# xiph/LPCNet

Hardware: AMD Instinct MI355X
Metric: 16 kHz samples/sec & concurrent real-time streams, 1/2/4/8 MI355X (higher is better)
Workload: dtype f32; 1 GPU; 2048 concurrent streams (each with its own feature file) per GPU x 25 frames (4000 samples) per step, fp32 weights, register-resident block-sparse GRU-A, bit-exact (PARITY) arithmetic; eight streams per CU as two groups of four half a step apart (BASELINE config 2's 1024 streams fill half of these stream slots: `also.config2_1024_streams`); arithmetic=parity, gru_a_blocks=1382, gru_a_densities=0.05,0.05,0.2 (benchmark model), gru_a_items_per_lane=30, streams_per_gpu=2048, streams_per_workgroup=8

## Files before the change

lpcnet_amd/csrc/sample_common.hip.h:

```cpp
#pragma once
#include <hip/hip_runtime.h>
#include <stdint.h>
#include "lpcnet_engine.h"
#include "lpcnet_math.h"

namespace lpcn {

constexpr int NA = LPCN_N_A, NB = LPCN_N_B, RA = LPCN_ROWS_A, RB = LPCN_ROWS_B;

#define LPCN_GLOBAL __attribute__((address_space(1)))
template <typename T> __device__ __forceinline__ const LPCN_GLOBAL T *as_global(const T *p)
{
    return (const LPCN_GLOBAL T *)(uintptr_t)p;
}
template <typename T> __device__ __forceinline__ LPCN_GLOBAL T *as_global_rw(T *p)
{
    return (LPCN_GLOBAL T *)(uintptr_t)p;
}
#define LPCN_REMAT_V(x) asm volatile("" : "+v"(x))
#define LPCN_REMAT_S(x) asm volatile("" : "+s"(x))

__device__ __forceinline__ uint32_t lds_addr(const void *ptr)
{
    return (uint32_t)(uintptr_t)(__attribute__((address_space(3))) unsigned char *)(unsigned char *)ptr;
}
__device__ __forceinline__ void lds_publish(const uint32_t addr, const int seq)
{
    asm volatile("ds_write_b32 %0, %1" :: "v"(addr), "v"(seq) : "memory");
}
__device__ __forceinline__ void lds_arrive(const uint32_t addr)
{
    int one = 1;
    unsigned long long ex;
    asm volatile("s_mov_b64 %0, exec\n\t"
                 "s_mov_b64 exec, 1\n\t"
                 "ds_add_u32 %1, %2\n\t"
                 "s_mov_b64 exec, %0"
                 : "=&s"(ex) : "v"(addr), "v"(one) : "memory");
}
template <bool SLEEP> __device__ __forceinline__ void lds_poll_until(const uint32_t addr, const int want)
{
    int v;
    do {
        asm volatile("ds_read_b32 %0, %1\n\ts_waitcnt lgkmcnt(0)" : "=v"(v) : "v"(addr) : "memory");
        v = __builtin_amdgcn_readfirstlane(v);
        if (SLEEP && v != want) __builtin_amdgcn_s_sleep(1);
    } while (v != want);
}


template <int J> __device__ __forceinline__ float row_bcast(float v)
{
    return __builtin_bit_cast(float, __builtin_amdgcn_update_dpp(0, __builtin_bit_cast(int, v), 0x150 + J, 0xf, 0xf, false));
}
template <int J> __device__ __forceinline__ float lpc_chain(float r, float prod)
{
    if constexpr (J < LPCN_LPC_ORDER) return lpc_chain<J + 1>(r - row_bcast<J>(prod), prod);
    else return r;
}
__device__ __forceinline__ float row_shr1(float v, float fill)
{
    return __builtin_bit_cast(float, __builtin_amdgcn_update_dpp(__builtin_bit_cast(int, fill), __builtin_bit_cast(int, v), 0x111, 0xf, 0xf, false));
}

struct LeaderCells {
    float *lead;
    int *idx;
    float *thr;
    short *pcm;
};

template <int S> __device__ __forceinline__ void open_sample(const LeaderCells &c, const int tid0, const bool live, const float newest, const float prod, const int exc, const bool per_frame)
{
    int t_ = tid0;
    LPCN_REMAT_V(t_);
    const int lrow = (t_ & 63) >> 4, tap = t_ & 15;
    const float r = lpc_chain<0>(0.f, prod);
    const int u = lpcn_lin2ulaw((tap & 1) ? r : newest);
    const int u_pred = __builtin_amdgcn_mov_dpp(u, 0xB1, 0xf, 0xf, true);
    if (tap == 0) {
        if (live) {
            c.lead[lrow * 8 + 0] = r;
            c.idx[lrow] = u | (u_pred << 8) | (exc << 16);
        } else {
            c.idx[lrow] = 0;
        }
        if (per_frame) c.idx[S + lrow] = live ? 1 : 0;
    }
}

__device__ __forceinline__ void draw_thresholds(const LeaderCells &c, const float *logit_tab, const int ls)
{
    int *li = (int *)c.lead + ls * 8;
    uint32_t rng[4] = {(uint32_t)li[4], (uint32_t)li[5], (uint32_t)li[6], (uint32_t)li[7]};
    const uint32_t r0 = lpcn_kiss99(rng), r1 = lpcn_kiss99(rng);
    li[4] = (int)rng[0]; li[5] = (int)rng[1]; li[6] = (int)rng[2]; li[7] = (int)rng[3];
#pragma unroll
    for (int b = 0; b < 4; ++b) {
        c.thr[ls * 8 + b] = logit_tab[(r0 >> (8 * b)) & 0xFF];
        c.thr[ls * 8 + 4 + b] = logit_tab[(r1 >> (8 * b)) & 0xFF];
    }
}

__device__ __forceinline__ int tree_walk(const unsigned long long *mask_row)
{
    typedef unsigned u4 __attribute__((ext_vector_type(4)));
    const u4 *mk = (const u4 *)mask_row;
    const u4 qa = mk[0], qb = mk[1], qc = mk[2], qd = mk[3];
    auto bit_of = [](unsigned word, int k) { return (int)((word >> (2 * k)) & 1u); };
    int val = 0;
#pragma unroll
    for (int b = 0; b < 4; ++b) val = (val << 1) | bit_of(qa[0], (1 << b) | val);
    val = (val << 1) | bit_of(qa[1], val);
    val = (val << 1) | bit_of((val & 16) ? qa[3] : qa[2], val & 15);
    {
        const int k = val >> 4;
        const unsigned lo = (k & 1) ? qb[1] : qb[0], hi = (k & 1) ? qb[3] : qb[2];
        val = (val << 1) | bit_of((k & 2) ? hi : lo, val & 15);
    }
    {
        const int k = val >> 4;
        const unsigned a0 = (k & 1) ? qc[1] : qc[0], a1 = (k & 1) ? qc[3] : qc[2];
        const unsigned a2 = (k & 1) ? qd[1] : qd[0], a3 = (k & 1) ? qd[3] : qd[2];
        const unsigned b0 = (k & 2) ? a1 : a0, b1 = (k & 2) ? a3 : a2;
        val = (val << 1) | bit_of((k & 4) ? b1 : b0, val & 15);
    }
    return val;
}

__device__ __forceinline__ void draw_sample(const LeaderCells &c, const unsigned long long *mask_row, const float *ulaw_tab, const int lrow, const int tap,
                                            const bool live, const int smp, const int preload, float &hist, float &pcm, float &deemph, int &exc)
{
    pcm = 0.f; deemph = 0.f; exc = 0;
    if (live) {
        const float pred = c.lead[lrow * 8 + 0];
        deemph = c.lead[lrow * 8 + 1];
        exc = tree_walk(mask_row);
        if (smp < preload) {
            const float x = (float)c.pcm[lrow * LPCN_FRAME_SIZE + smp];
            exc = lpcn_lin2ulaw(x - 0.85f * deemph - pred);
            pcm = x - 0.85f * deemph;
        } else {
            pcm = pred + ulaw_tab[exc];
        }
    }
    {
        const float shifted = row_shr1(hist, pcm);
        hist = live ? shifted : hist;
    }
    if (tap == 0 && live) ((int *)c.lead)[lrow * 8 + 2] = exc;
}
__device__ __forceinline__ void finish_sample(const LeaderCells &c, const int lrow, const int tap, const bool live, const int smp, const int preload, float pcm, const float deemph)
{
    if (tap == 0) {
        if (live) {
            pcm = pcm + 0.85f * deemph;
            c.lead[lrow * 8 + 1] = pcm;
            if (smp >= preload) c.pcm[lrow * LPCN_FRAME_SIZE + smp] = (short)lpcn_round_pcm(pcm);
        } else {
            c.pcm[lrow * LPCN_FRAME_SIZE + smp] = 0;
        }
    }
}
__device__ __forceinline__ bool stream_is_live(const LpcnSampleArgs *Ap, const LPCN_GLOBAL lpcn_stream_state *states, const int stream, const int f)
{
    const int fc_ref = Ap->fc_base ? as_global(Ap->fc_base)[stream] : states[stream].frame_count;
    int fc = Ap->fc_advance ? fc_ref + f + 1 : fc_ref;
    if (fc > 1000) fc = 1000;
    return fc > LPCN_FEATURES_DELAY;
}

template <class L> __device__ __forceinline__ void stage_tables(unsigned char *smem, const LpcnSampleArgs *Ap, const int tid, const int brec_dwords)
{
    const auto *t0 = as_global(Ap->tab_tansig), *t1 = as_global(Ap->tab_ulaw2lin), *t2 = as_global(Ap->tab_logit);
    for (int i = tid; i < 201; i += LPCN_WG_THREADS) ((float *)(smem + L::tansig))[i] = t0[i];
    for (int i = tid; i < 256; i += LPCN_WG_THREADS) {
        ((float *)(smem + L::ulaw))[i] = t1[i];
        ((float *)(smem + L::logit))[i] = t2[i];
    }
    const auto *ab1 = as_global(Ap->a_bias1), *adg = as_global(Ap->a_diag);
    for (int i = tid; i < RA; i += LPCN_WG_THREADS) {
        ((float *)(smem + L::abias))[2 * i] = ab1[i];
        ((float *)(smem + L::abias))[2 * i + 1] = adg[i];
    }
    const auto *br = as_global(Ap->b_rec), *bb = as_global(Ap->b_bias);
    for (int i = tid; i < brec_dwords; i += LPCN_WG_THREADS) ((uint32_t *)(smem + L::brec))[i] = ((const LPCN_GLOBAL uint32_t *)br)[i];
    for (int i = tid; i < 2 * RB; i += LPCN_WG_THREADS) ((float *)(smem + L::bbias))[i] = bb[i];
    if (tid < 7) ((int *)(smem + L::bstart))[tid] = as_global(Ap->b_start)[tid];
}
#define LPCN_GRUB_SHIFT 0x321100
__device__ __forceinline__ void stage_grub_weights(unsigned char *bw, const LpcnSampleArgs *Ap, const int tid, const bool shifted)
{
    const int nb_b = Ap->nb_b;
    const auto *src = (const LPCN_GLOBAL uint32_t *)as_global(Ap->b_w);
    for (int i = tid; i < (nb_b + 8) * 32; i += LPCN_WG_THREADS) {
        int di = i;
        if (shifted) {
            if (i < nb_b * 32) di = i + ((LPCN_GRUB_SHIFT >> (4 * ((i >> 5) / 96))) & 15) * 32;
            else if (i < (nb_b + 5) * 32) di = i + 3 * 32;
            else continue;
        }
        ((uint32_t *)bw)[di] = i < nb_b * 32 ? src[i] : 0u;
    }
}
__device__ __forceinline__ void stage_leader_record(const LeaderCells &c, const int s, const LPCN_GLOBAL lpcn_stream_state *st)
{
    c.idx[s] = 0;
    c.lead[s * 8 + 0] = 0.f;
    c.lead[s * 8 + 1] = st->deemph_mem;
    ((int *)c.lead)[s * 8 + 2] = st->last_exc;
#pragma unroll
    for (int j = 0; j < 4; ++j) ((uint32_t *)c.lead)[s * 8 + 4 + j] = st->rng[j];
}
}
```

lpcnet_amd/csrc/sample_kernel_x2.hip.h:

```cpp
#pragma once
#include "sample_kernel.hip.h"

namespace lpcn {

#define LPCN_X2_LW 4
#define LPCN_X2_TW 0
#define LPCN_X2_HG 10

struct LdsX2 {
    static constexpr int S = 4;
    static constexpr int HA_STRIDE = 16 * S;
    static constexpr int g_hA    = 0;
    static constexpr int g_hT    = g_hA + 96 * HA_STRIDE + 24 * 16;
    static constexpr int g_prec  = g_hT + NA * S * 4;
    static constexpr int g_hB    = g_prec + NA * S * 4;
    static constexpr int g_idx   = g_hB + S * NB * 4;
    static constexpr int g_thr   = g_idx + S * 16;
    static constexpr int g_mask  = g_thr + S * 32;
    static constexpr int g_lead  = g_mask + S * 64;
    static constexpr int g_flag  = g_lead + S * 32;
    static constexpr int g_condb = g_flag + 16;
    static constexpr int g_lpc   = g_condb + S * RB * 4;
    static constexpr int g_pcm   = g_lpc + S * 64;
    static constexpr int G_SZ    = g_pcm + S * 320;
    static constexpr int pre_ur  = 2 * G_SZ;
    static constexpr int inh     = pre_ur + 2 * NA * S * 4;
    static constexpr int abias   = inh + NA * S * 4;
    static constexpr int tansig  = abias + 2 * RA * 4;
    static constexpr int ulaw    = tansig + 816;
    static constexpr int logit   = ulaw + 1024;
    static constexpr int brec    = logit + 1024;
    static constexpr int bbias   = brec + NB * RB * 4;
    static constexpr int bstart  = bbias + 2 * RB * 4;
    static constexpr int bw      = bstart + 32;
    static constexpr int total(int nb_b) { return bw + (nb_b + 8) * 128; }
    __host__ __device__ static constexpr int ha_off(int p) { return p * HA_STRIDE + (p >> 2) * 16; }
};

template <int NW>
__global__ __launch_bounds__(LPCN_WG_THREADS, 2) void sample_kernel_x2(const LpcnSampleArgs *__restrict__ Ap)
{
    using L = LdsX2;
    constexpr int S = 4;
    constexpr int LW = LPCN_X2_LW, TW = LPCN_X2_TW;
    extern __shared__ __attribute__((aligned(16))) unsigned char smem[];
    float *const sm_pre_ur = (float *)(smem + L::pre_ur);
    float *const sm_inh = (float *)(smem + L::inh);
    const float *const sm_abias = (const float *)(smem + L::abias);
    const float *const sm_tansig = (const float *)(smem + L::tansig);
    const float *const sm_ulaw = (const float *)(smem + L::ulaw);
    const float *const sm_logit = (const float *)(smem + L::logit);
    const float *const sm_brec = (const float *)(smem + L::brec);
    const float *const sm_bbias = (const float *)(smem + L::bbias);
    const int *const sm_bstart = (const int *)(smem + L::bstart);

    const int tid0 = threadIdx.x;
    const int n_streams = Ap->n_streams, n_frames = Ap->n_frames, preload = Ap->preload, frame_len = Ap->frame_len;
    const int s0 = blockIdx.x * 2 * S;
    auto stream_of = [&](int gs) __attribute__((always_inline)) { return (s0 + gs < n_streams) ? s0 + gs : n_streams - 1; };
    const int n_valid = (n_streams - s0 < 2 * S) ? n_streams - s0 : 2 * S;
    const size_t nf = (size_t)n_frames;
    auto *const states = as_global_rw(Ap->state);
    const LPCN_GLOBAL float *emb_nat_sig = as_global(Ap->emb_nat_sig), *emb_nat_pred = as_global(Ap->emb_nat_pred), *emb_nat_exc = as_global(Ap->emb_nat_exc);
    asm volatile("" : "+s"(emb_nat_sig), "+s"(emb_nat_pred), "+s"(emb_nat_exc));

    float4 w[NW];
    uint32_t offp[(NW + 1) / 2];
    int row_reg[3];
#define LPCN_ROW(k) (row_reg[k])
    {
        const int lane = tid0 & 63, wave = tid0 >> 6;
        const size_t base = (size_t)wave * NW * 64 + lane;
        const int lane_sel = (lane & 3) * 16;
        const auto *ab = as_global(Ap->a_blk);
        const auto *aw = (const LPCN_GLOBAL float *)as_global(Ap->a_w);
#pragma unroll
        for (int j = 0; j < NW; ++j) {
            const auto *v = aw + (base + (size_t)j * 64) * 4;
            w[j] = make_float4(v[0], v[1], v[2], v[3]);
        }
#pragma unroll
        for (int j = 0; j < NW; j += 2) {
            const int p0 = ab[base + (size_t)j * 64];
            const int p1 = (j + 1 < NW) ? ab[base + (size_t)(j + 1) * 64] : 0;
            offp[j >> 1] = (uint32_t)(L::ha_off(p0) + lane_sel) | ((uint32_t)(L::ha_off(p1) + lane_sel) << 16);
        }
        const auto *ar = as_global(Ap->a_row);
#pragma unroll
        for (int k = 0; k < 3; ++k) row_reg[k] = ar[(wave * 3 + k) * 64 + lane];
    }
    int b1 = __builtin_amdgcn_readfirstlane(as_global(Ap->a_bound)[(tid0 >> 6) * 4 + 1]);
    int b2 = __builtin_amdgcn_readfirstlane(as_global(Ap->a_bound)[(tid0 >> 6) * 4 + 2]);
    int b3 = __builtin_amdgcn_readfirstlane(as_global(Ap->a_bound)[(tid0 >> 6) * 4 + 3]);
    const bool allh0 = __builtin_amdgcn_readfirstlane(as_global(Ap->a_allh)[(tid0 >> 6) * 3]) != 0;
    const LPCN_GLOBAL float *fc_w_s = as_global(Ap->fc_w), *fc_b_s = as_global(Ap->fc_b), *fc_f_s = as_global(Ap->fc_f);
    asm volatile("" : "+s"(fc_w_s), "+s"(fc_b_s), "+s"(fc_f_s));
    const LPCN_GLOBAL float *cond_a_s = as_global(Ap->cond_a);
    asm volatile("" : "+s"(cond_a_s));
    const int has_slot = __builtin_amdgcn_readfirstlane((__ballot(row_reg[0] >= 0) != 0ull ? 1 : 0) | (__ballot(row_reg[1] >= 0) != 0ull ? 2 : 0) |
                                                        (__ballot(row_reg[2] >= 0) != 0ull ? 4 : 0));
    const bool has2 = (has_slot & 4) != 0;
    const int hl = __builtin_amdgcn_readfirstlane(as_global(Ap->a_head)[tid0 >> 6]);
    const bool early_wave = hl > 0;
    const bool plain_start = __builtin_amdgcn_readfirstlane(((early_wave || __ballot(row_reg[0] >= 2 * NA) == 0ull) && __ballot(row_reg[1] >= 2 * NA || row_reg[2] >= 2 * NA) == 0ull) ? 1 : 0) != 0;

    {
        const int tid = tid0;
        stage_tables<L>(smem, Ap, tid, NB * RB);
        stage_grub_weights(smem + L::bw, Ap, tid, true);
        for (int i = tid; i < 2 * S * NA; i += LPCN_WG_THREADS) {
            const int gs = i / NA, n = i % NA, g = gs >> 2, s = gs & 3;
            const float hv0 = states[stream_of(gs)].gru_a[n];
            unsigned char *gb = smem + g * L::G_SZ;
            ((float *)(gb + L::g_hT))[n * S + s] = hv0;
            *(float *)(gb + L::g_hA + L::ha_off(n >> 2) + s * 16 + (n & 3) * 4) = hv0;
        }
        for (int i = tid; i < 2 * S * NB; i += LPCN_WG_THREADS) {
            const int gs = i / NB, g = gs >> 2, s = gs & 3;
            ((float *)(smem + g * L::G_SZ + L::g_hB))[s * NB + i % NB] = states[stream_of(gs)].gru_b[i % NB];
        }
        if (tid < 2 * S) {
            const int g = tid >> 2, s = tid & 3;
            unsigned char *gb = smem + g * L::G_SZ;
            stage_leader_record({(float *)(gb + L::g_lead), (int *)(gb + L::g_idx), nullptr, nullptr}, s, &states[stream_of(tid)]);
        }
        if (tid < 2) { int *fl = (int *)(smem + tid * L::G_SZ + L::g_flag); fl[0] = 0; fl[1] = 0; fl[2] = 0; }
    }
    __syncthreads();

    const bool is_lw = (tid0 >> 6) == LW;
    const bool is_tw_lane = tid0 >= 64 * TW && tid0 < 64 * TW + S;
#define LPCN_LROW ((tid0 & 63) >> 4)
#define LPCN_TAP (tid0 & 15)
    float histP = is_lw ? states[stream_of(S + LPCN_LROW)].last_sig[LPCN_TAP] : 0.f;
    float histQ = is_lw ? states[stream_of(LPCN_LROW)].last_sig[LPCN_TAP] : 0.f;
    bool liveP = false, liveQ = false;
    int live_maskP = 0, live_maskQ = 0;
    int seqP = 0, seqQ = 0;
    int chnP = 0, chnQ = 0;
    int smpP = 0, smpQ = 0, fP = 0, fQ = 0;
    float lpc_tap = 0.f, prod_old = 0.f;

    const int T = n_frames * frame_len;
#if LPCN_ENABLE_PROF
#ifndef LPCN_PROF_MASK
#define LPCN_PROF_MASK 0xFFF
#endif
    unsigned long long *const prof = Ap->prof;
    unsigned long long pt[12] = {0, 0, 0, 0, 0, 0, 0, 0, 0, 0, 0, 0}, tprev = 0;
    const bool profiling = prof != nullptr && blockIdx.x == 0;
#define LPCN_X2_PROF(slot) do { if (((LPCN_PROF_MASK >> (slot)) & 1) && profiling) { const unsigned long long now_ = __builtin_amdgcn_s_memtime(); pt[slot] += now_ - tprev; tprev = now_; } } while (0)
    if (profiling) tprev = __builtin_amdgcn_s_memtime();
#else
#define LPCN_X2_PROF(slot) do { } while (0)
#endif
    for (int h = -1; h <= 2 * T + 1; ++h) {
        const int p = h & 1, q = p ^ 1;
        unsigned char *const gp = smem + p * L::G_SZ, *const gq = smem + q * L::G_SZ;
        const bool p_active = h >= 0 && (h >> 1) < T;
        const bool p_prev = h >= 2;
        const bool q_chain = h >= 1 && ((h - 1) >> 1) < T;
        const bool q_heads = ((h + 1) >> 1) < T;
        const bool new_frame = p_active && smpP == 0;
        const bool more = p_active && smpP != 0;
        float *const hT_p = (float *)(gp + L::g_hT);
        float *const hB_q = (float *)(gq + L::g_hB);
        int *const idx_p = (int *)(gp + L::g_idx);
        float *const lpc_p = (float *)(gp + L::g_lpc);
        short *const pcm_p = (short *)(gp + L::g_pcm);
        const LeaderCells cells_p = {(float *)(gp + L::g_lead), idx_p, (float *)(gp + L::g_thr), pcm_p};
        const uint32_t flag_p = lds_addr(gp + L::g_flag);

        if (more) ++seqP;
        if (p_prev && is_lw) {
            __builtin_amdgcn_s_setprio(3);
            const int smp_done = smpP == 0 ? frame_len - 1 : smpP - 1;
            int t_ = tid0;
            LPCN_REMAT_V(t_);
            const int lrow = (t_ & 63) >> 4, tap = t_ & 15;
            float pcm, deemph;
            int exc;
            draw_sample(cells_p, (const unsigned long long *)(gp + L::g_mask) + lrow * 8, sm_ulaw, lrow, tap, liveP, smp_done, preload, histP, pcm, deemph, exc);
            if (more) { open_sample<S>(cells_p, tid0, liveP, pcm, tap == 0 ? pcm * lpc_tap : prod_old, exc, false); lds_publish(flag_p, seqP); }
            __builtin_amdgcn_s_setprio(0);
            finish_sample(cells_p, lrow, tap, liveP, smp_done, preload, pcm, deemph);
        }
        if (more && is_tw_lane && liveP) { int t_ = tid0; LPCN_REMAT_V(t_); draw_thresholds(cells_p, sm_logit, t_ - 64 * TW); }

        if (new_frame) {
            int tid = tid0;
            LPCN_REMAT_V(tid);
            const bool lw_ = (tid >> 6) == LW, twl_ = tid >= 64 * TW && tid < 64 * TW + S;
            __syncthreads();
            if (fP > 0) {
                auto *out = as_global_rw(Ap->pcm);
                const size_t pstride = (size_t)Ap->pcm_stride;
                for (int i = tid; i < S * LPCN_FRAME_SIZE; i += LPCN_WG_THREADS) {
                    const int s = i / LPCN_FRAME_SIZE, k = i % LPCN_FRAME_SIZE;
                    if (S * p + s < n_valid && k < frame_len) out[(size_t)(s0 + S * p + s) * pstride + (size_t)(fP - 1) * LPCN_FRAME_SIZE + k] = pcm_p[i];
                }
            }
            __syncthreads();
            {
                const auto *cb = as_global(Ap->cond_b), *lp = as_global(Ap->lpc);
                float *const condb_p = (float *)(gp + L::g_condb);
                if (tid < S * RB) condb_p[tid] = cb[((size_t)stream_of(S * p + tid / RB) * nf + fP) * RB + tid % RB];
                if (tid >= 256 && tid < 256 + S * LPCN_LPC_ORDER) {
                    const int i = tid - 256;
                    lpc_p[i] = lp[((size_t)stream_of(S * p + i / LPCN_LPC_ORDER) * nf + fP) * LPCN_LPC_ORDER + i % LPCN_LPC_ORDER];
                }
                if (lw_ || twl_) {
                    const int lstream = stream_of(S * p + (lw_ ? (tid & 63) >> 4 : tid - 64 * TW));
                    liveP = stream_is_live(Ap, states, lstream, fP);
                }
                if (preload > 0 && tid < S) {
                    const auto *pin = as_global(Ap->pcm) + (size_t)stream_of(S * p + tid) * (size_t)Ap->pcm_stride + (size_t)fP * LPCN_FRAME_SIZE;
                    for (int i = 0; i < preload; ++i) pcm_p[tid * LPCN_FRAME_SIZE + i] = pin[i];
                }
            }
            __syncthreads();
            ++seqP;
            if (lw_) {
                open_sample<S>(cells_p, tid0, liveP, histP, histP * lpc_p[tid & 63], ((const int *)cells_p.lead)[((tid & 63) >> 4) * 8 + 2], true);
                lds_publish(flag_p, seqP);
            }
            if (twl_ && liveP) draw_thresholds(cells_p, sm_logit, tid - 64 * TW);
            __syncthreads();
            int lm = 0;
#pragma unroll
            for (int s = 0; s < S; ++s) lm |= (idx_p[S + s] ? 1 : 0) << s;
            live_maskP = __builtin_amdgcn_readfirstlane(lm);
        }

        LPCN_X2_PROF(0);
        float acc[S] = {};
        constexpr int PF = 2;
        float4 hq[PF + 1] = {};
        const unsigned char *hA_cur = gp + L::g_hA;
        auto fetch_h = [&](const int j) __attribute__((always_inline)) {
            uint32_t pk = offp[j >> 1];
            LPCN_REMAT_V(pk);
            const uint32_t off = (j & 1) ? (pk >> 16) : (pk & 0xFFFFu);
            hq[j % (PF + 1)] = *(const float4 *)(hA_cur + off);
        };
        typedef float negz_t __attribute__((ext_vector_type(4)));
        negz_t negz = {-0.f, -0.f, -0.f, -0.f};
        auto load_negz = [&]() __attribute__((always_inline)) { negz = (negz_t){-0.f, -0.f, -0.f, -0.f}; asm volatile("" : "+v"(negz)); };
        auto mac = [&](const int j) __attribute__((always_inline)) {
            typedef float f4 __attribute__((ext_vector_type(4)));
            typedef float f2 __attribute__((ext_vector_type(2)));
            const float4 hv = hq[j % (PF + 1)];
            const float hk[4] = {hv.x, hv.y, hv.z, hv.w};
            const float wk[4] = {w[j].x, w[j].y, w[j].z, w[j].w};
            f2 a01 = {acc[0], acc[1]}, a23 = {acc[2], acc[3]};
            f4 pv[4];
#pragma unroll
            for (int c = 0; c < 4; ++c) pv[c] = __builtin_amdgcn_mfma_f32_4x4x1f32(hk[c], wk[c], negz, 0, 0, 0);
            __builtin_amdgcn_sched_barrier(0);
#pragma unroll
            for (int c = 0; c < 4; ++c) {
                a01 = a01 + __builtin_shufflevector(pv[c], pv[c], 0, 1);
                a23 = a23 + __builtin_shufflevector(pv[c], pv[c], 2, 3);
            }
            acc[0] = a01[0]; acc[1] = a01[1]; acc[2] = a23[0]; acc[3] = a23[1];
        };
        auto pre_cell = [&](const int r, unsigned char *gb) __attribute__((always_inline)) -> float * {
            return (float *)(r < 2 * NA ? smem + L::pre_ur + r * (S * 4) : gb + L::g_prec + (r - 2 * NA) * (S * 4));
        };

        const int lane = tid0 & 63;
        const int wave = __builtin_amdgcn_readfirstlane(tid0 >> 6);
        float fcw[NB], fcb = 0.f, fcf = 0.f;
        auto load_fc = [&]() __attribute__((always_inline)) {
            int t_ = tid0;
            LPCN_REMAT_V(t_);
            const int node_ = t_ >> 1, chan_ = t_ & 1;
            const auto *fcw_ptr = fc_w_s + node_ * 2 * NB + chan_ * NB;
#pragma unroll
            for (int j = 0; j < NB; ++j) fcw[j] = fcw_ptr[j];
            fcb = fc_b_s[chan_ * 256 + node_]; fcf = fc_f_s[chan_ * 256 + node_];
        };
        const uint32_t chcnt_q = lds_addr(gq + L::g_flag) + 8;
        if (q_chain) ++chnQ;

        constexpr int J0 = NW - LPCN_EARLY_MAX < 0 ? 0 : NW - LPCN_EARLY_MAX;
        constexpr int JM = J0 + LPCN_X2_HG < NW ? J0 + LPCN_X2_HG : NW;
        const bool do_heads = early_wave && q_heads;
        int e0 = NW - hl;
        LPCN_REMAT_S(e0);
        auto head_step = [&](auto self, auto jc, auto jend_c) __attribute__((always_inline)) -> void {
            constexpr int j = decltype(jc)::value, je = decltype(jend_c)::value;
            if constexpr (j < je) {
                if constexpr (j + PF < NW) fetch_h(j + PF);
                if (j >= e0) { asm volatile(""); mac(j); }
                self(self, std::integral_constant<int, j + 1>{}, jend_c);
            }
        };
        const uint32_t p0cnt_p = flag_p + 4;
        constexpr int CW = LPCN_X2_CHAIN_WAVES, P0W = LPCN_X2_P0_FIRST, NP0 = LPCN_WAVES - P0W;
        static_assert(NP0 * 64 * 3 == 2 * NA && CW == S, "three rounds of the row waves' lanes cover GRU-A's update / reset rows");
        const bool p0_wave = p_active && wave >= P0W;
        uint32_t o_sig[S] = {}, o_pred[S] = {}, o_exc[S] = {}, o_cond[S] = {};
        constexpr int P0PERM = 0x3102;
        int i0 = 0;
        float ld[3][4 * S] = {};
        auto p0_open = [&]() __attribute__((always_inline)) {
            int gi[S];
            {
                typedef int i4 __attribute__((ext_vector_type(4)));
                i4 v;
                int f;
                const uint32_t idx_a = lds_addr(idx_p);
                do {
                    asm volatile("ds_read_b32 %0, %2\n\tds_read_b128 %1, %3\n\ts_waitcnt lgkmcnt(0)" : "=&v"(f), "=&v"(v) : "v"(flag_p), "v"(idx_a) : "memory");
                    f = __builtin_amdgcn_readfirstlane(f);
                } while (f != seqP);
#pragma unroll
                for (int s = 0; s < S; ++s) gi[s] = __builtin_amdgcn_readfirstlane(v[s]);
            }
#pragma unroll
            for (int s = 0; s < S; ++s) {
                o_sig[s] = (uint32_t)(gi[s] & 0xFF) * (uint32_t)(RA * 4);
                o_pred[s] = (uint32_t)((gi[s] >> 8) & 0xFF) * (uint32_t)(RA * 4);
                o_exc[s] = ((uint32_t)(gi[s] >> 16) & 0xFFu) * (uint32_t)(RA * 4);
                o_cond[s] = (uint32_t)(((size_t)stream_of(S * p + s) * nf + (size_t)fP) * RA * 4);
            }
            int t_ = tid0;
            LPCN_REMAT_V(t_);
            i0 = (((P0PERM >> (4 * ((t_ >> 6) & 3))) & 3) << 6) | (t_ & 63);
        };
        const bool fifth = ((P0PERM >> (4 * (wave & 3))) & 3) < 2;
        auto issue = [&](const int k, const int buf) __attribute__((always_inline)) {
            const uint32_t rb = (uint32_t)(i0 + 256 * k) * 4u;
#pragma unroll
            for (int s = 0; s < S; ++s) {
                ld[buf][4 * s + 0] = *(const LPCN_GLOBAL float *)((const LPCN_GLOBAL char *)cond_a_s + (o_cond[s] + rb));
                ld[buf][4 * s + 1] = *(const LPCN_GLOBAL float *)((const LPCN_GLOBAL char *)emb_nat_sig + (o_sig[s] + rb));
                ld[buf][4 * s + 2] = *(const LPCN_GLOBAL float *)((const LPCN_GLOBAL char *)emb_nat_pred + (o_pred[s] + rb));
                ld[buf][4 * s + 3] = *(const LPCN_GLOBAL float *)((const LPCN_GLOBAL char *)emb_nat_exc + (o_exc[s] + rb));
            }
        };
        auto reduce = [&](const int k, const int buf) __attribute__((always_inline)) {
            const int r = i0 + 256 * k;
            float g[S];
#pragma unroll
            for (int s = 0; s < S; ++s) g[s] = ((ld[buf][4 * s + 0] + ld[buf][4 * s + 1]) + ld[buf][4 * s + 2]) + ld[buf][4 * s + 3];
            if (k < 3) {
                const int n = r >= NA ? r - NA : r;
                const float2 bd = *(const float2 *)(sm_abias + 2 * r);
                const float4 hv = *(const float4 *)(hT_p + n * S);
                *(float4 *)(sm_pre_ur + r * S) = make_float4((bd.x + bd.y * hv.x) + g[0], (bd.x + bd.y * hv.y) + g[1], (bd.x + bd.y * hv.z) + g[2], (bd.x + bd.y * hv.w) + g[3]);
            } else {
                *(float4 *)(sm_inh + (r - 2 * NA) * S) = make_float4(g[0], g[1], g[2], g[3]);
            }
        };
        if (wave < CW) {
            if (q_chain) {
                __builtin_amdgcn_s_setprio(3);
                const int s = wave;
                int ln_ = tid0;
                LPCN_REMAT_V(ln_);
                ln_ &= 63;
                const int r = ln_ < RB ? ln_ : RB - 1;
                const int g6 = r >> 3, ri = r & 7;
                const float *const condb_q = (const float *)(gq + L::g_condb);
                float zrh = sm_bbias[r] + condb_q[s * RB + r];
                float rec = sm_bbias[RB + r];
#pragma unroll
                for (int j = 0; j < NB; ++j) rec = rec + sm_brec[j * RB + r] * hB_q[s * NB + j];
                uint32_t wp32 = lds_addr(smem + L::bw + (sm_bstart[g6] * 8 + ri) * 16 + ((LPCN_GRUB_SHIFT >> (4 * g6)) & 15) * 128);
                uint32_t hp32 = lds_addr(gq + L::g_hA + s * 16);
                asm volatile(
#include "grub_lds_loop_s4.inc"
                    : [z] "+v"(zrh), [wp] "+v"(wp32), [hp] "+v"(hp32) : : LPCN_GRUB_LDS_CLOBBERS);
                __builtin_amdgcn_s_setprio(0);
                LPCN_X2_PROF(1);
                const int ln = ln_ & 15;
                const float sg = lpcn_sigmoid(zrh + rec, sm_tansig);
                const float r_gate = __builtin_bit_cast(float, __builtin_amdgcn_ds_bpermute((16 + ln) << 2, __builtin_bit_cast(int, sg)));
                const float hc = lpcn_tanh(zrh + rec * r_gate, sm_tansig);
                const float hc_i = __builtin_bit_cast(float, __builtin_amdgcn_ds_bpermute((32 + ln) << 2, __builtin_bit_cast(int, hc)));
                if (ln_ < NB) {
                    const float hold = hB_q[s * NB + ln_];
                    const float hnew = sg * hold + (1.f - sg) * hc_i;
                    if ((live_maskQ >> s) & 1) hB_q[s * NB + ln_] = hnew;
                }
                lds_arrive(chcnt_q);
                LPCN_X2_PROF(2);
            }
        } else {
            if (do_heads) {
                hA_cur = gq + L::g_hA;
                load_negz();
                {
                    int r = LPCN_ROW(0);
                    LPCN_REMAT_V(r);
                    r = r < 0 ? 0 : r;
                    const int n = r - 2 * NA;
                    const float bias = sm_abias[2 * r], diag = sm_abias[2 * r + 1];
                    const float *hT_q = (const float *)(gq + L::g_hT);
#pragma unroll
                    for (int s = 0; s < S; ++s) acc[s] = bias + diag * hT_q[n * S + s];
                }
#pragma unroll
                for (int j = 0; j < PF; ++j) if (J0 + j < NW) fetch_h(J0 + j);
                head_step(head_step, std::integral_constant<int, J0>{}, std::integral_constant<int, JM>{});
            }
            LPCN_X2_PROF(3);
            if (p0_wave) {
                p0_open();
                LPCN_X2_PROF(1);
                issue(0, 0); issue(1, 1); issue(2, 2);
                LPCN_X2_PROF(2);
                reduce(0, 0); reduce(1, 1); reduce(2, 2);
                lds_arrive(p0cnt_p);
                issue(3, 0);
                if (fifth) issue(4, 1);
            }
            LPCN_X2_PROF(4);
            if (do_heads) {
                head_step(head_step, std::integral_constant<int, JM>{}, std::integral_constant<int, NW>{});
                int r = LPCN_ROW(0);
                LPCN_REMAT_V(r);
                if (r >= 0) {
                    float *c = pre_cell(r, gq);
#pragma unroll
                    for (int s = 0; s < S; ++s) c[s] = acc[s];
                }
            }
            if (p0_wave) { reduce(3, 0); if (fifth) reduce(4, 1); }
            LPCN_X2_PROF(3);
        }

        if (p_active) {
            hA_cur = gp + L::g_hA;
            load_negz();
            lds_poll_until<false>(p0cnt_p, seqP * NP0);
            LPCN_X2_PROF(11);
            if (plain_start) {
                int r = LPCN_ROW(0);
                LPCN_REMAT_V(r);
                r = r < 0 ? 0 : r;
                const float *c = pre_cell(r, gp);
#pragma unroll
                for (int s = 0; s < S; ++s) acc[s] = c[s];
            } else {
#pragma unroll
            for (int k = 0; k < 3; ++k) {
                int r = LPCN_ROW(k);
                LPCN_REMAT_V(r);
                const bool live_row = r >= 0;
                r = r < 0 ? 0 : r;
                const bool candidate = r >= 2 * NA;
                const int n = candidate ? r - 2 * NA : 0;
                const float bias = sm_abias[2 * r], diag = sm_abias[2 * r + 1];
                float *c = pre_cell(r, gp);
                const bool parked = k == 0 && early_wave;
#pragma unroll
                for (int s = 0; s < S; ++s) {
                    const float bv = bias + diag * hT_p[n * S + s];
                    if (k == 0) acc[s] = (candidate && !parked) ? bv : c[s];
                    else if (candidate && live_row) c[s] = bv;
                }
            }
            }
            auto row_swap = [&](const int k_done, const int k_next) __attribute__((always_inline)) {
                int r = LPCN_ROW(k_done), r2 = LPCN_ROW(k_next);
                LPCN_REMAT_V(r);
                LPCN_REMAT_V(r2);
                if (r >= 0) {
                    float *c = pre_cell(r, gp);
#pragma unroll
                    for (int s = 0; s < S; ++s) c[s] = acc[s];
                }
                r2 = r2 < 0 ? 0 : r2;
                const float *c2 = pre_cell(r2, gp);
#pragma unroll
                for (int s = 0; s < S; ++s) acc[s] = c2[s];
            };
            auto row_store = [&](const int k) __attribute__((always_inline)) {
                int r = LPCN_ROW(k);
                LPCN_REMAT_V(r);
                if (r >= 0) {
                    float *c = pre_cell(r, gp);
#pragma unroll
                    for (int s = 0; s < S; ++s) c[s] = acc[s];
                }
            };
            const int jend = b3;
            LPCN_X2_PROF(4);
#pragma unroll
            for (int j = 0; j < PF && j < NW; ++j) fetch_h(j);
            LPCN_REMAT_S(b1);
            LPCN_REMAT_S(b2);
            LPCN_REMAT_S(b3);
            int nextb = b1;
            LPCN_REMAT_S(nextb);
            auto item = [&](const int j) __attribute__((always_inline)) -> bool {
                if (__builtin_expect(j >= jend, 0)) return false;
                if (j + PF < NW) fetch_h(j + PF);
                if (__builtin_expect(j == nextb, 0)) {
                    if (j == b1) row_swap(0, 1);
                    if (j == b2) row_swap(1, 2);
                    __builtin_amdgcn_s_waitcnt(0xC07F);
                    nextb = b1 > j ? b1 : (b2 > j ? b2 : NW);
                }
                mac(j);
                return true;
            };
            auto run_items = [&](auto self, auto jc) __attribute__((always_inline)) -> void {
                constexpr int j = decltype(jc)::value;
                if constexpr (j < NW) {
                    if (!item(j)) return;
                    self(self, std::integral_constant<int, j + 1>{});
                }
            };
            run_items(run_items, std::integral_constant<int, 0>{});
            if (q_chain) load_fc();
            LPCN_X2_PROF(5);
            if (b1 >= jend) {
                row_swap(0, 1);
                row_swap(1, 2);
                row_store(2);
            } else if (b2 >= jend) {
                row_swap(1, 2);
                row_store(2);
            } else {
                row_store(2);
            }
            LPCN_X2_PROF(6);
        }
        if (q_chain) {
            if (!p_active) load_fc();
            lds_poll_until<false>(chcnt_q, chnQ * S);
            int tid = tid0;
            LPCN_REMAT_V(tid);
            const int node = tid >> 1;
            const int node_level = node > 0 ? 31 - __clz(node) : 0;
            const float *const thr_q = (const float *)(gq + L::g_thr);
            unsigned long long *const mask_q = (unsigned long long *)(gq + L::g_mask);
            float sums[S];
            {
                typedef float f4 __attribute__((ext_vector_type(4)));
                typedef float f2 __attribute__((ext_vector_type(2)));
                float hs[NB];
                const float4 *hp = (const float4 *)(hB_q + (tid & 3) * NB);
#pragma unroll
                for (int qd = 0; qd < NB / 4; ++qd) { const float4 v4 = hp[qd]; hs[4 * qd] = v4.x; hs[4 * qd + 1] = v4.y; hs[4 * qd + 2] = v4.z; hs[4 * qd + 3] = v4.w; }
                load_negz();
                f2 s01 = {fcb, fcb}, s23 = {fcb, fcb};
#pragma unroll
                for (int jb = 0; jb < NB; jb += 4) {
                    f4 pv[4];
#pragma unroll
                    for (int c = 0; c < 4; ++c) pv[c] = __builtin_amdgcn_mfma_f32_4x4x1f32(hs[jb + c], fcw[jb + c], negz, 0, 0, 0);
                    __builtin_amdgcn_sched_barrier(0);
#pragma unroll
                    for (int c = 0; c < 4; ++c) {
                        s01 = s01 + __builtin_shufflevector(pv[c], pv[c], 0, 1);
                        s23 = s23 + __builtin_shufflevector(pv[c], pv[c], 2, 3);
                    }
                }
                sums[0] = s01[0]; sums[1] = s01[1]; sums[2] = s23[0]; sums[3] = s23[1];
            }
            float vq[S], thq[S];
            unsigned long long mq[S];
#pragma unroll
            for (int s = 0; s < S; ++s) { vq[s] = lpcn_tanh(sums[s], sm_tansig); thq[s] = thr_q[s * 8 + node_level]; }
#pragma unroll
            for (int s = 0; s < S; ++s) {
                const float v = fcf * vq[s];
                const float vo = __builtin_bit_cast(float, __builtin_amdgcn_mov_dpp(__builtin_bit_cast(int, v), 0xB1, 0xf, 0xf, true));
                const float lg = v + vo;
                mq[s] = __ballot(thq[s] < lg) & (wave == 0 ? 0x5555555555555554ull : 0x5555555555555555ull);
            }
            if (lane == 0) {
#pragma unroll
                for (int s = 0; s < S; ++s) mask_q[s * 8 + wave] = mq[s];
            }
            if (is_lw) {
                lpc_tap = ((const float *)(gq + L::g_lpc))[tid & 63];
                prod_old = row_shr1(histQ, 0.f) * lpc_tap;
            }
        }
        LPCN_X2_PROF(9);
        __syncthreads();
        LPCN_X2_PROF(7);

        int tid = tid0;
        LPCN_REMAT_V(tid);
        if (p_active) {
            constexpr int NI = NA * S, NQ = NI / LPCN_WG_THREADS;
            const float *const prec_p = (const float *)(gp + L::g_prec);
            float z[NQ], rg[NQ], a[NQ], hold[NQ];
#pragma unroll
            for (int k = 0; k < NQ; ++k) {
                const int i = tid + k * LPCN_WG_THREADS;
                z[k] = sm_pre_ur[i];
                rg[k] = sm_pre_ur[NI + i];
                a[k] = prec_p[i];
                hold[k] = hT_p[i];
            }
#pragma unroll
            for (int k = 0; k < NQ; ++k) { z[k] = lpcn_sigmoid(z[k], sm_tansig); rg[k] = lpcn_sigmoid(rg[k], sm_tansig); }
#pragma unroll
            for (int k = 0; k < NQ; ++k) a[k] = a[k] * rg[k] + sm_inh[tid + k * LPCN_WG_THREADS];
#pragma unroll
            for (int k = 0; k < NQ; ++k) a[k] = lpcn_tanh(a[k], sm_tansig);
            const unsigned ut = (unsigned)tid;
            const bool live_s = ((live_maskP >> (ut & 3u)) & 1) != 0;
            unsigned char *const ha0 = gp + L::g_hA + L::ha_off((int)(ut >> 4)) + (ut & 3u) * 16u + ((ut >> 2) & 3u) * 4u;
            static_assert(L::ha_off(32) == 32 * L::HA_STRIDE + 8 * 16 && LPCN_WG_THREADS == 512 && S == 4, "gate-stage address stride");
#pragma unroll
            for (int k = 0; k < NQ; ++k) {
                const float hnew = z[k] * hold[k] + (1.f - z[k]) * a[k];
                const float hv = live_s ? hnew : hold[k];
                hT_p[tid + k * LPCN_WG_THREADS] = hv;
                *(float *)(ha0 + k * L::ha_off(32)) = hv;
            }
        }
        LPCN_X2_PROF(8);
        __syncthreads();
        LPCN_X2_PROF(10);

        if (p_active) { if (++smpP == frame_len) { smpP = 0; ++fP; } }
        { const float t = histP; histP = histQ; histQ = t; }
        { const bool t = liveP; liveP = liveQ; liveQ = t; }
        { const int t = live_maskP; live_maskP = live_maskQ; live_maskQ = t; }
        { const int t = seqP; seqP = seqQ; seqQ = t; }
        { const int t = chnP; chnP = chnQ; chnQ = t; }
        { const int t = smpP; smpP = smpQ; smpQ = t; }
        { const int t = fP; fP = fQ; fQ = t; }
        asm volatile("; LPCN_SAMPLE_LOOP_END" ::: "memory");
        __builtin_amdgcn_sched_barrier(0);
    }

#if LPCN_ENABLE_PROF
    if (profiling && (tid0 & 63) == 0) {
#pragma unroll
        for (int i = 0; i < 12; ++i) prof[(tid0 >> 6) * 12 + i] += pt[i];
    }
#endif
    __syncthreads();
    {
        auto *out = as_global_rw(Ap->pcm);
        const size_t pstride = (size_t)Ap->pcm_stride;
        for (int i = tid0; i < 2 * S * LPCN_FRAME_SIZE; i += LPCN_WG_THREADS) {
            const int gs = i / LPCN_FRAME_SIZE, k = i % LPCN_FRAME_SIZE;
            const short *pb = (const short *)(smem + (gs >> 2) * L::G_SZ + L::g_pcm);
            if (gs < n_valid && k < frame_len) out[(size_t)(s0 + gs) * pstride + (size_t)(n_frames - 1) * LPCN_FRAME_SIZE + k] = pb[(gs & 3) * LPCN_FRAME_SIZE + k];
        }
    }
    {
        const int tid = tid0;
        for (int i = tid; i < 2 * S * NA; i += LPCN_WG_THREADS) {
            const int gs = i / NA, n = i % NA;
            if (gs < n_valid) states[s0 + gs].gru_a[n] = ((const float *)(smem + (gs >> 2) * L::G_SZ + L::g_hT))[n * S + (gs & 3)];
        }
        for (int i = tid; i < 2 * S * NB; i += LPCN_WG_THREADS) {
            const int gs = i / NB;
            if (gs < n_valid) states[s0 + gs].gru_b[i % NB] = ((const float *)(smem + (gs >> 2) * L::G_SZ + L::g_hB))[(gs & 3) * NB + i % NB];
        }
        if (is_lw) {
            if (LPCN_LROW < n_valid) states[s0 + LPCN_LROW].last_sig[LPCN_TAP] = histP;
            if (S + LPCN_LROW < n_valid) states[s0 + S + LPCN_LROW].last_sig[LPCN_TAP] = histQ;
        }
        if (tid < n_valid) {
            auto *st = &states[s0 + tid];
            const unsigned char *gb = smem + (tid >> 2) * L::G_SZ;
            const int *li = (const int *)(gb + L::g_lead) + (tid & 3) * 8;
            const float *lp = (const float *)(gb + L::g_lpc);
#pragma unroll
            for (int j = 0; j < LPCN_LPC_ORDER; ++j) st->lpc[j] = lp[(tid & 3) * LPCN_LPC_ORDER + j];
            st->deemph_mem = ((const float *)li)[1];
            st->last_exc = li[2];
#pragma unroll
            for (int j = 0; j < 4; ++j) st->rng[j] = (uint32_t)li[4 + j];
        }
    }
#undef LPCN_ROW
#undef LPCN_LROW
#undef LPCN_TAP
}

}
```

Measured before the change: 159.3 million samples/s.

## Replace full 256-node sampling tree evaluation with two-stage per-stream walk

Drops the old chain stage, which evaluated all 255 tree nodes for four streams with MFMA after a counter-based LDS wait and then walked the ballot mask. Each stream's wave now evaluates only the 31 top-level nodes, walks them, loads the 7 nodes of the selected subtree, and writes the final 8-bit sample index to LDS. The leader reads that index directly instead of walking a mask. This removes most of the FC dot products and the arrival counter, but puts a dependent second weight load from global memory and two serial ballot walks on the GRU-B critical path.

```diff
diff --git a/lpcnet_amd/csrc/sample_common.hip.h b/lpcnet_amd/csrc/sample_common.hip.h
--- a/lpcnet_amd/csrc/sample_common.hip.h
+++ b/lpcnet_amd/csrc/sample_common.hip.h
@@ -128,14 +128,15 @@
     return val;
 }
 
-__device__ __forceinline__ void draw_sample(const LeaderCells &c, const unsigned long long *mask_row, const float *ulaw_tab, const int lrow, const int tap,
-                                            const bool live, const int smp, const int preload, float &hist, float &pcm, float &deemph, int &exc)
+template <class Walked>
+__device__ __forceinline__ void draw_sample_with(const LeaderCells &c, const Walked walked, const float *ulaw_tab, const int lrow, const int tap,
+                                                 const bool live, const int smp, const int preload, float &hist, float &pcm, float &deemph, int &exc)
 {
     pcm = 0.f; deemph = 0.f; exc = 0;
     if (live) {
         const float pred = c.lead[lrow * 8 + 0];
         deemph = c.lead[lrow * 8 + 1];
-        exc = tree_walk(mask_row);
+        exc = walked();
         if (smp < preload) {
             const float x = (float)c.pcm[lrow * LPCN_FRAME_SIZE + smp];
             exc = lpcn_lin2ulaw(x - 0.85f * deemph - pred);
@@ -149,6 +150,16 @@
         hist = live ? shifted : hist;
     }
     if (tap == 0 && live) ((int *)c.lead)[lrow * 8 + 2] = exc;
+}
+__device__ __forceinline__ void draw_sample(const LeaderCells &c, const unsigned long long *mask_row, const float *ulaw_tab, const int lrow, const int tap,
+                                            const bool live, const int smp, const int preload, float &hist, float &pcm, float &deemph, int &exc)
+{
+    draw_sample_with(c, [&]() { return tree_walk(mask_row); }, ulaw_tab, lrow, tap, live, smp, preload, hist, pcm, deemph, exc);
+}
+__device__ __forceinline__ void draw_sample_walked(const LeaderCells &c, const int *walked_cell, const float *ulaw_tab, const int lrow, const int tap,
+                                                   const bool live, const int smp, const int preload, float &hist, float &pcm, float &deemph, int &exc)
+{
+    draw_sample_with(c, [&]() { return *walked_cell & 0xFF; }, ulaw_tab, lrow, tap, live, smp, preload, hist, pcm, deemph, exc);
 }
 __device__ __forceinline__ void finish_sample(const LeaderCells &c, const int lrow, const int tap, const bool live, const int smp, const int preload, float pcm, const float deemph)
 {
diff --git a/lpcnet_amd/csrc/sample_kernel_x2.hip.h b/lpcnet_amd/csrc/sample_kernel_x2.hip.h
--- a/lpcnet_amd/csrc/sample_kernel_x2.hip.h
+++ b/lpcnet_amd/csrc/sample_kernel_x2.hip.h
@@ -1,5 +1,6 @@
 #pragma once
 #include "sample_kernel.hip.h"
+#include "tree_stages.h"
 
 namespace lpcn {
 
@@ -37,6 +38,41 @@
     __host__ __device__ static constexpr int ha_off(int p) { return p * HA_STRIDE + (p >> 2) * 16; }
 };
 
+typedef float tree_f4 __attribute__((ext_vector_type(4)));
+struct TreeRow { tree_f4 w[NB / 4]; float bias, factor; };
+template <int STAGE>
+__device__ __forceinline__ TreeRow tree_row_load(const LPCN_GLOBAL float *fc_w, const LPCN_GLOBAL float *fc_b, const LPCN_GLOBAL float *fc_f, const int lane, const int prefix)
+{
+    const int node = lpcn_tree_node(STAGE, lpcn_tree_lane_local(STAGE, lane), prefix), chan = lane & 1;
+    const auto *wp = (const LPCN_GLOBAL tree_f4 *)(fc_w + (node * 2 + chan) * NB);
+    TreeRow r;
+#pragma unroll
+    for (int j = 0; j < NB / 4; ++j) r.w[j] = wp[j];
+    r.bias = fc_b[chan * 256 + node];
+    r.factor = fc_f[chan * 256 + node];
+    return r;
+}
+template <int STAGE>
+__device__ __forceinline__ int tree_stage_walk(const TreeRow &r, const float *h_s, const float *thr_s, const float *tansig, const int lane)
+{
+    const float4 *hp = (const float4 *)h_s;
+    float sum = r.bias;
+#pragma unroll
+    for (int j = 0; j < NB / 4; ++j) {
+        const float4 hv = hp[j];
+        const tree_f4 wv = r.w[j];
+        sum = sum + wv[0] * hv.x;
+        sum = sum + wv[1] * hv.y;
+        sum = sum + wv[2] * hv.z;
+        sum = sum + wv[3] * hv.w;
+    }
+    const float v = r.factor * lpcn_tanh(sum, tansig);
+    const float vo = __builtin_bit_cast(float, __builtin_amdgcn_mov_dpp(__builtin_bit_cast(int, v), 0xB1, 0xf, 0xf, true));
+    const float lg = v + vo;
+    const unsigned long long m = __ballot(thr_s[lpcn_tree_level(STAGE, lpcn_tree_lane_local(STAGE, lane))] < lg) & lpcn_tree_stage_mask(STAGE);
+    return lpcn_tree_stage_walk(m, STAGE == 0 ? LPCN_TREE_TOP : LPCN_TREE_LEVELS - LPCN_TREE_TOP);
+}
+
 template <int NW>
 __global__ __launch_bounds__(LPCN_WG_THREADS, 2) void sample_kernel_x2(const LpcnSampleArgs *__restrict__ Ap)
 {
@@ -124,7 +160,7 @@
             unsigned char *gb = smem + g * L::G_SZ;
             stage_leader_record({(float *)(gb + L::g_lead), (int *)(gb + L::g_idx), nullptr, nullptr}, s, &states[stream_of(tid)]);
         }
-        if (tid < 2) { int *fl = (int *)(smem + tid * L::G_SZ + L::g_flag); fl[0] = 0; fl[1] = 0; fl[2] = 0; }
+        if (tid < 2) { int *fl = (int *)(smem + tid * L::G_SZ + L::g_flag); fl[0] = 0; fl[1] = 0; }
     }
     __syncthreads();
 
@@ -137,7 +173,6 @@
     bool liveP = false, liveQ = false;
     int live_maskP = 0, live_maskQ = 0;
     int seqP = 0, seqQ = 0;
-    int chnP = 0, chnQ = 0;
     int smpP = 0, smpQ = 0, fP = 0, fQ = 0;
     float lpc_tap = 0.f, prod_old = 0.f;
 
@@ -180,7 +215,7 @@
             const int lrow = (t_ & 63) >> 4, tap = t_ & 15;
             float pcm, deemph;
             int exc;
-            draw_sample(cells_p, (const unsigned long long *)(gp + L::g_mask) + lrow * 8, sm_ulaw, lrow, tap, liveP, smp_done, preload, histP, pcm, deemph, exc);
+            draw_sample_walked(cells_p, (const int *)(gp + L::g_mask) + lrow, sm_ulaw, lrow, tap, liveP, smp_done, preload, histP, pcm, deemph, exc);
             if (more) { open_sample<S>(cells_p, tid0, liveP, pcm, tap == 0 ? pcm * lpc_tap : prod_old, exc, false); lds_publish(flag_p, seqP); }
             __builtin_amdgcn_s_setprio(0);
             finish_sample(cells_p, lrow, tap, liveP, smp_done, preload, pcm, deemph);
@@ -268,20 +303,7 @@
             return (float *)(r < 2 * NA ? smem + L::pre_ur + r * (S * 4) : gb + L::g_prec + (r - 2 * NA) * (S * 4));
         };
 
-        const int lane = tid0 & 63;
         const int wave = __builtin_amdgcn_readfirstlane(tid0 >> 6);
-        float fcw[NB], fcb = 0.f, fcf = 0.f;
-        auto load_fc = [&]() __attribute__((always_inline)) {
-            int t_ = tid0;
-            LPCN_REMAT_V(t_);
-            const int node_ = t_ >> 1, chan_ = t_ & 1;
-            const auto *fcw_ptr = fc_w_s + node_ * 2 * NB + chan_ * NB;
-#pragma unroll
-            for (int j = 0; j < NB; ++j) fcw[j] = fcw_ptr[j];
-            fcb = fc_b_s[chan_ * 256 + node_]; fcf = fc_f_s[chan_ * 256 + node_];
-        };
-        const uint32_t chcnt_q = lds_addr(gq + L::g_flag) + 8;
-        if (q_chain) ++chnQ;
 
         constexpr int J0 = NW - LPCN_EARLY_MAX < 0 ? 0 : NW - LPCN_EARLY_MAX;
         constexpr int JM = J0 + LPCN_X2_HG < NW ? J0 + LPCN_X2_HG : NW;
@@ -375,6 +397,7 @@
                     : [z] "+v"(zrh), [wp] "+v"(wp32), [hp] "+v"(hp32) : : LPCN_GRUB_LDS_CLOBBERS);
                 __builtin_amdgcn_s_setprio(0);
                 LPCN_X2_PROF(1);
+                const TreeRow top = tree_row_load<0>(fc_w_s, fc_b_s, fc_f_s, ln_, 0);
                 const int ln = ln_ & 15;
                 const float sg = lpcn_sigmoid(zrh + rec, sm_tansig);
                 const float r_gate = __builtin_bit_cast(float, __builtin_amdgcn_ds_bpermute((16 + ln) << 2, __builtin_bit_cast(int, sg)));
@@ -385,8 +408,13 @@
                     const float hnew = sg * hold + (1.f - sg) * hc_i;
                     if ((live_maskQ >> s) & 1) hB_q[s * NB + ln_] = hnew;
                 }
-                lds_arrive(chcnt_q);
                 LPCN_X2_PROF(2);
+                const float *const thr_s = (const float *)(gq + L::g_thr) + s * 8;
+                int val = tree_stage_walk<0>(top, hB_q + s * NB, thr_s, sm_tansig, ln_);
+                const TreeRow sub = tree_row_load<1>(fc_w_s, fc_b_s, fc_f_s, ln_, val);
+                val = (val << (LPCN_TREE_LEVELS - LPCN_TREE_TOP)) | tree_stage_walk<1>(sub, hB_q + s * NB, thr_s, sm_tansig, ln_);
+                if (ln_ == 0) ((int *)(gq + L::g_mask))[s] = val;
+                LPCN_X2_PROF(9);
             }
         } else {
             if (do_heads) {
@@ -516,7 +544,6 @@
                 }
             };
             run_items(run_items, std::integral_constant<int, 0>{});
-            if (q_chain) load_fc();
             LPCN_X2_PROF(5);
             if (b1 >= jend) {
                 row_swap(0, 1);
@@ -530,58 +557,11 @@
             }
             LPCN_X2_PROF(6);
         }
-        if (q_chain) {
-            if (!p_active) load_fc();
-            lds_poll_until<false>(chcnt_q, chnQ * S);
-            int tid = tid0;
-            LPCN_REMAT_V(tid);
-            const int node = tid >> 1;
-            const int node_level = node > 0 ? 31 - __clz(node) : 0;
-            const float *const thr_q = (const float *)(gq + L::g_thr);
-            unsigned long long *const mask_q = (unsigned long long *)(gq + L::g_mask);
-            float sums[S];
-            {
-                typedef float f4 __attribute__((ext_vector_type(4)));
-                typedef float f2 __attribute__((ext_vector_type(2)));
-                float hs[NB];
-                const float4 *hp = (const float4 *)(hB_q + (tid & 3) * NB);
-#pragma unroll
-                for (int qd = 0; qd < NB / 4; ++qd) { const float4 v4 = hp[qd]; hs[4 * qd] = v4.x; hs[4 * qd + 1] = v4.y; hs[4 * qd + 2] = v4.z; hs[4 * qd + 3] = v4.w; }
-                load_negz();
-                f2 s01 = {fcb, fcb}, s23 = {fcb, fcb};
-#pragma unroll
-                for (int jb = 0; jb < NB; jb += 4) {
-                    f4 pv[4];
-#pragma unroll
-                    for (int c = 0; c < 4; ++c) pv[c] = __builtin_amdgcn_mfma_f32_4x4x1f32(hs[jb + c], fcw[jb + c], negz, 0, 0, 0);
-                    __builtin_amdgcn_sched_barrier(0);
-#pragma unroll
-                    for (int c = 0; c < 4; ++c) {
-                        s01 = s01 + __builtin_shufflevector(pv[c], pv[c], 0, 1);
-                        s23 = s23 + __builtin_shufflevector(pv[c], pv[c], 2, 3);
-                    }
-                }
-                sums[0] = s01[0]; sums[1] = s01[1]; sums[2] = s23[0]; sums[3] = s23[1];
-            }
-            float vq[S], thq[S];
-            unsigned long long mq[S];
-#pragma unroll
-            for (int s = 0; s < S; ++s) { vq[s] = lpcn_tanh(sums[s], sm_tansig); thq[s] = thr_q[s * 8 + node_level]; }
-#pragma unroll
-            for (int s = 0; s < S; ++s) {
-                const float v = fcf * vq[s];
-                const float vo = __builtin_bit_cast(float, __builtin_amdgcn_mov_dpp(__builtin_bit_cast(int, v), 0xB1, 0xf, 0xf, true));
-                const float lg = v + vo;
-                mq[s] = __ballot(thq[s] < lg) & (wave == 0 ? 0x5555555555555554ull : 0x5555555555555555ull);
-            }
-            if (lane == 0) {
-#pragma unroll
-                for (int s = 0; s < S; ++s) mask_q[s * 8 + wave] = mq[s];
-            }
-            if (is_lw) {
-                lpc_tap = ((const float *)(gq + L::g_lpc))[tid & 63];
-                prod_old = row_shr1(histQ, 0.f) * lpc_tap;
-            }
+        if (q_chain && is_lw) {
+            int t_ = tid0;
+            LPCN_REMAT_V(t_);
+            lpc_tap = ((const float *)(gq + L::g_lpc))[t_ & 63];
+            prod_old = row_shr1(histQ, 0.f) * lpc_tap;
         }
         LPCN_X2_PROF(9);
         __syncthreads();
@@ -628,7 +608,6 @@
         { const bool t = liveP; liveP = liveQ; liveQ = t; }
         { const int t = live_maskP; live_maskP = live_maskQ; live_maskQ = t; }
         { const int t = seqP; seqP = seqQ; seqQ = t; }
-        { const int t = chnP; chnP = chnQ; chnQ = t; }
         { const int t = smpP; smpP = smpQ; smpQ = t; }
         { const int t = fP; fP = fQ; fQ = t; }
         asm volatile("; LPCN_SAMPLE_LOOP_END" ::: "memory");
diff --git a/lpcnet_amd/csrc/tree_stages.h b/lpcnet_amd/csrc/tree_stages.h
--- /dev/null
+++ b/lpcnet_amd/csrc/tree_stages.h
@@ -0,0 +1,29 @@
+#pragma once
+#include "lpcnet_math.h"
+
+#define LPCN_TREE_LEVELS 8
+#define LPCN_TREE_TOP 5
+
+LPCN_HD constexpr int lpcn_tree_stage_nodes(const int stage) { return stage == 0 ? (1 << LPCN_TREE_TOP) - 1 : (1 << (LPCN_TREE_LEVELS - LPCN_TREE_TOP)) - 1; }
+LPCN_HD constexpr int lpcn_tree_lane_local(const int stage, const int lane)
+{
+    const int k = lane >> 1;
+    return (k >= 1 && k <= lpcn_tree_stage_nodes(stage)) ? k : 1;
+}
+LPCN_HD constexpr int lpcn_tree_local_level(const int k) { return k >= 16 ? 4 : k >= 8 ? 3 : k >= 4 ? 2 : k >= 2 ? 1 : 0; }
+LPCN_HD constexpr int lpcn_tree_level(const int stage, const int k) { return (stage == 0 ? 0 : LPCN_TREE_TOP) + lpcn_tree_local_level(k); }
+LPCN_HD constexpr int lpcn_tree_node(const int stage, const int k, const int prefix)
+{
+    const int l = lpcn_tree_local_level(k), root = stage == 0 ? 1 : (1 << LPCN_TREE_TOP) | prefix;
+    return (root << l) | (k - (1 << l));
+}
+LPCN_HD constexpr unsigned long long lpcn_tree_stage_mask(const int stage)
+{
+    return 0x5555555555555555ull & ((1ull << (2 * lpcn_tree_stage_nodes(stage) + 1)) - 1) & ~3ull;
+}
+LPCN_HD constexpr int lpcn_tree_stage_walk(const unsigned long long ballot, const int levels)
+{
+    int val = 0;
+    for (int b = 0; b < levels; ++b) val = (val << 1) | (int)((ballot >> (2 * ((1 << b) | val))) & 1ull);
+    return val;
+}
```

After: 163.2 million samples/s (median of 6 runs). 1.02x the previous value.
